# SpectacularAI/HybVIO

Measured on AMD Instinct MI355X. Metric: VIO frames/sec at 752x480 stereo, 200 KLT features; pyramid+KLT HBM GB/s, higher is better.
Workload: dtype u8/int16 pixels, int32/int64 sums, f32 solve (tracker); f64 (EKF); 1 GPU; C3: 752x480 stereo, 200 pts -- the whole frame chained on one stream per sequence: 2 pyramid builds, temporal LK from predicted positions, 2-point rotation RANSAC on its output, stereo LK, GFTT key points every 2nd frame (HIP tracker), then the HIP EKF from the device mean: 20 track visits (triangulation + prepareVisualUpdate + chi2 gate; track lengths 5 + Geometric(0.2) <= 21 stereo poses = 20 .~; sequences_per_gpu=4096, engines_per_gpu=4, parallelism=replicas x1 (no collective)

## Files before the change

hybvio_amd/csrc/rot_ransac.hip:

```cpp
#include "hv_camera.hpp"
#include "hv_internal.hpp"

#include <algorithm>
#include <cmath>

namespace hv {
namespace {

constexpr int RT_MANY = 256;
constexpr int RT_FEW = 1024;
constexpr int MAX_PTS = 1024;
constexpr int HYP = 100;
constexpr int RT_SPLIT_GROUPS = 25, RT_SPLIT = 256;
static_assert(HYP % RT_SPLIT_GROUPS == 0, "whole groups of hypotheses");
constexpr size_t SPLIT_REC_BYTES = sizeof(int) * (2 * HYP + 4) + sizeof(float) * 9 * HYP;

struct RansacArgs {
    int max_points;
    const int *n_points;
    const float *c1, *c2;
    const int *pairs;
    const uint32_t *draws;
    const uint8_t *lk_status;
    int lk_tracked;
    float threshold_pow2;
    int *status;
    float *R;
    int *summary;
    unsigned char *split;
    hv_camera_model cam1, cam2;
};

__device__ void cross3(const double *a, const double *b, double *c)
{
    c[0] = a[1] * b[2] - a[2] * b[1]; c[1] = a[2] * b[0] - a[0] * b[2]; c[2] = a[0] * b[1] - a[1] * b[0];
}

template <int P, int Q>
__device__ __forceinline__ void jacobi_step(double *A, double *V)
{
    const double apq = A[3 * P + Q];
    if (apq == 0.0) return;
    const double theta = (A[3 * Q + Q] - A[3 * P + P]) / (2.0 * apq);
    const double t = (theta >= 0.0 ? 1.0 : -1.0) / (fabs(theta) + sqrt(theta * theta + 1.0));
    const double c = 1.0 / sqrt(t * t + 1.0), s = t * c;
#pragma unroll
    for (int k = 0; k < 3; ++k) {
        const double akp = A[3 * k + P], akq = A[3 * k + Q];
        A[3 * k + P] = c * akp - s * akq; A[3 * k + Q] = s * akp + c * akq;
    }
#pragma unroll
    for (int k = 0; k < 3; ++k) {
        const double apk = A[3 * P + k], aqk = A[3 * Q + k];
        A[3 * P + k] = c * apk - s * aqk; A[3 * Q + k] = s * apk + c * aqk;
    }
#pragma unroll
    for (int k = 0; k < 3; ++k) {
        const double vkp = V[3 * k + P], vkq = V[3 * k + Q];
        V[3 * k + P] = c * vkp - s * vkq; V[3 * k + Q] = s * vkp + c * vkq;
    }
}

__device__ void kabsch_rotation(const float *Hf, float *Rf)
{
    double H[9], A[9], V[9] = {1, 0, 0, 0, 1, 0, 0, 0, 1};
#pragma unroll
    for (int k = 0; k < 9; ++k) H[k] = (double)Hf[k];
#pragma unroll
    for (int r = 0; r < 3; ++r)
#pragma unroll
        for (int c = 0; c < 3; ++c) A[3 * r + c] = H[r] * H[c] + H[3 + r] * H[3 + c] + H[6 + r] * H[6 + c];
    for (int sweep = 0; sweep < 8; ++sweep) { jacobi_step<0, 1>(A, V); jacobi_step<0, 2>(A, V); jacobi_step<1, 2>(A, V); }
    const double e0 = A[0], e1 = A[4], e2 = A[8];
    int i0 = 0;
    if (e1 > e0) i0 = 1;
    if (e2 > (i0 == 0 ? e0 : e1)) i0 = 2;
    auto eig = [&](int i) { return i == 0 ? e0 : i == 1 ? e1 : e2; };
    int i1 = i0 == 0 ? 1 : 0;
#pragma unroll
    for (int k = 0; k < 3; ++k) if (k != i0 && eig(k) > eig(i1)) i1 = k;
    auto col = [&](int i, int r) { return i == 0 ? V[3 * r] : i == 1 ? V[3 * r + 1] : V[3 * r + 2]; };
    const double v1[3] = {col(i0, 0), col(i0, 1), col(i0, 2)}, v2[3] = {col(i1, 0), col(i1, 1), col(i1, 2)};
    double v3[3], u1[3], u2[3], u3[3];
    const double l1 = eig(i0), l2 = eig(i1);
    const double s1 = sqrt(l1 > 0 ? l1 : 0.0), s2 = sqrt(l2 > 0 ? l2 : 0.0);
#pragma unroll
    for (int r = 0; r < 3; ++r) {
        u1[r] = H[3 * r] * v1[0] + H[3 * r + 1] * v1[1] + H[3 * r + 2] * v1[2];
        u2[r] = H[3 * r] * v2[0] + H[3 * r + 1] * v2[1] + H[3 * r + 2] * v2[2];
    }
    if (s1 > 0.0) {
#pragma unroll
        for (int r = 0; r < 3; ++r) u1[r] /= s1;
    } else { u1[0] = 1; u1[1] = 0; u1[2] = 0; }
    if (s2 > 1e-12 * s1 && s2 > 0.0) {
        const double d = u2[0] * u1[0] + u2[1] * u1[1] + u2[2] * u1[2];
#pragma unroll
        for (int r = 0; r < 3; ++r) u2[r] = u2[r] / s2 - (d / s2) * u1[r];
        const double nn = sqrt(u2[0] * u2[0] + u2[1] * u2[1] + u2[2] * u2[2]);
#pragma unroll
        for (int r = 0; r < 3; ++r) u2[r] /= nn;
    } else {
        int k0 = 0;
        if (fabs(u1[1]) < fabs(u1[0])) k0 = 1;
        if (fabs(u1[2]) < fabs(k0 == 0 ? u1[0] : u1[1])) k0 = 2;
        const double ax2[3] = {k0 == 0 ? 1.0 : 0.0, k0 == 1 ? 1.0 : 0.0, k0 == 2 ? 1.0 : 0.0};
        cross3(u1, ax2, u2);
        const double nn = sqrt(u2[0] * u2[0] + u2[1] * u2[1] + u2[2] * u2[2]);
#pragma unroll
        for (int r = 0; r < 3; ++r) u2[r] /= nn;
    }
    cross3(v1, v2, v3);
    cross3(u1, u2, u3);
#pragma unroll
    for (int r = 0; r < 3; ++r)
#pragma unroll
        for (int c = 0; c < 3; ++c) Rf[3 * r + c] = (float)(v1[r] * u1[c] + v2[r] * u2[c] + v3[r] * u3[c]);
}

__device__ bool inlier(const float *R, const float *p1, float c2x, float c2y, const hv_camera_model &cam2, double thr)
{
    float q[3];
#pragma unroll
    for (int r = 0; r < 3; ++r) {
        float s = 0.0f;
#pragma unroll
        for (int k = 0; k < 3; ++k) s = s + R[3 * r + k] * p1[k];
        q[r] = s;
    }
    const double ray[3] = {(double)q[0], (double)q[1], (double)q[2]};
    double pix[2];
    if (!ray_to_pixel(cam2, ray, pix)) return false;
    const float qx = (float)pix[0], qy = (float)pix[1];
    const double dx = (double)(c2x - qx), dy = (double)(c2y - qy);
    return dx * dx + dy * dy <= thr;
}

template <int RT, int NG = 1>
__global__ __launch_bounds__(RT) void rot_ransac_kernel(RansacArgs a)
{
    constexpr int HPG = HYP / NG;
    __shared__ float s_p1[MAX_PTS * 3], s_p2[MAX_PTS * 3], s_c2[MAX_PTS * 2];
    __shared__ float s_R[HYP * 9];
    __shared__ int s_count[HYP], s_valid[HYP];
    __shared__ unsigned char s_in[MAX_PTS];
    __shared__ float s_Rb[9];
    __shared__ int s_best[4];
    __shared__ unsigned short s_map[MAX_PTS];
    __shared__ int s_chunk[MAX_PTS / 64 + 1];
    const int set = NG > 1 ? blockIdx.y : blockIdx.x, tid = threadIdx.x;
    const int k_lo = NG > 1 ? (int)blockIdx.x * HPG : 0;
    const int n_all = min(max(a.n_points[set], 0), a.max_points);
    const float *c1 = a.c1 + (size_t)set * a.max_points * 2, *c2 = a.c2 + (size_t)set * a.max_points * 2;
    int *status = a.status + (size_t)set * a.max_points;
    int n = n_all;
    if (a.lk_status) {
        const uint8_t *ls = a.lk_status + (size_t)set * a.max_points;
        const int nchunk = (n_all + 63) / 64, wave = tid >> 6, lane = tid & 63;
        for (int ch = wave; ch < nchunk; ch += RT / 64) {
            const int i = ch * 64 + lane;
            const unsigned long long m = __ballot(i < n_all && ls[i] == a.lk_tracked);
            if (lane == 0) s_chunk[ch] = __popcll(m);
        }
        __syncthreads();
        if (tid == 0) {
            int acc = 0;
            for (int ch = 0; ch < nchunk; ++ch) { const int cnt = s_chunk[ch]; s_chunk[ch] = acc; acc += cnt; }
            s_chunk[nchunk] = acc;
        }
        __syncthreads();
        n = s_chunk[nchunk];
        for (int ch = wave; ch < nchunk; ch += RT / 64) {
            const int i = ch * 64 + lane;
            const bool on = i < n_all && ls[i] == a.lk_tracked;
            const unsigned long long m = __ballot(on);
            if (on) s_map[s_chunk[ch] + __popcll(m & ((1ull << lane) - 1ull))] = (unsigned short)i;
        }
    } else {
        for (int i = tid; i < n_all; i += RT) s_map[i] = (unsigned short)i;
    }
    __syncthreads();
    if (n < 2) {
        if (tid == 0 && k_lo == 0) { a.summary[2 * set] = 0; a.summary[2 * set + 1] = 0; }
        return;
    }
    const double thr = (double)a.threshold_pow2;
    for (int i = tid; i < n; i += RT) {
        const int src = s_map[i];
        double r[3];
        pixel_to_ray(a.cam1, (double)c1[2 * src], (double)c1[2 * src + 1], r);
        s_p1[3 * i] = (float)r[0]; s_p1[3 * i + 1] = (float)r[1]; s_p1[3 * i + 2] = (float)r[2];
        pixel_to_ray(a.cam2, (double)c2[2 * src], (double)c2[2 * src + 1], r);
        s_p2[3 * i] = (float)r[0]; s_p2[3 * i + 1] = (float)r[1]; s_p2[3 * i + 2] = (float)r[2];
        s_c2[2 * i] = c2[2 * src]; s_c2[2 * i + 1] = c2[2 * src + 1];
    }
    if (tid < HYP) s_count[tid] = 0;
    __syncthreads();
    if (tid < HPG) {
        const int hk = k_lo + tid;
        int i1, i2;
        if (a.draws) {
            i1 = (int)(a.draws[((size_t)set * HYP + hk) * 2] % (uint32_t)n);
            i2 = (int)(a.draws[((size_t)set * HYP + hk) * 2 + 1] % (uint32_t)n);
        } else {
            i1 = a.pairs[((size_t)set * HYP + hk) * 2]; i2 = a.pairs[((size_t)set * HYP + hk) * 2 + 1];
        }
        const int ok = i1 != i2 && (unsigned)i1 < (unsigned)n && (unsigned)i2 < (unsigned)n;
        s_valid[hk] = ok;
        if (ok) {
            float H[9] = {0, 0, 0, 0, 0, 0, 0, 0, 0}, R[9];
#pragma unroll
            for (int w = 0; w < 2; ++w) {
                const float *p = s_p1 + 3 * (w ? i2 : i1), *q = s_p2 + 3 * (w ? i2 : i1);
#pragma unroll
                for (int r = 0; r < 3; ++r)
#pragma unroll
                    for (int c = 0; c < 3; ++c) { const float prod = p[r] * q[c]; H[3 * r + c] = H[3 * r + c] + prod; }
            }
            kabsch_rotation(H, R);
#pragma unroll
            for (int k = 0; k < 9; ++k) s_R[9 * hk + k] = R[k];
        }
    }
    __syncthreads();
    for (int w = tid; w < n * HPG; w += RT) {
        const int kk = w / n, i = w - kk * n, k = k_lo + kk;
        if (s_valid[k] && inlier(s_R + 9 * k, s_p1 + 3 * i, s_c2[2 * i], s_c2[2 * i + 1], a.cam2, thr)) atomicAdd(&s_count[k], 1);
    }
    __syncthreads();
    if constexpr (NG > 1) {
        int *rec_i = reinterpret_cast<int *>(a.split + (size_t)set * SPLIT_REC_BYTES);
        float *rec_R = reinterpret_cast<float *>(rec_i + 2 * HYP + 4);
        if (tid < HPG) {
            rec_i[k_lo + tid] = s_count[k_lo + tid];
            rec_i[HYP + k_lo + tid] = s_valid[k_lo + tid];
        }
        for (int i = tid; i < 9 * HPG; i += RT) rec_R[9 * k_lo + i] = s_valid[k_lo + i / 9] ? s_R[9 * k_lo + i] : 0.0f;
        __threadfence();
        __syncthreads();
        if (tid == 0) s_best[3] = atomicAdd(&rec_i[2 * HYP], 1);
        __syncthreads();
        if (s_best[3] != NG - 1) return;
        __threadfence();
        if (tid < HYP) {
            s_count[tid] = __hip_atomic_load(&rec_i[tid], __ATOMIC_RELAXED, __HIP_MEMORY_SCOPE_AGENT);
            s_valid[tid] = __hip_atomic_load(&rec_i[HYP + tid], __ATOMIC_RELAXED, __HIP_MEMORY_SCOPE_AGENT);
        }
        for (int i = tid; i < 9 * HYP; i += RT) s_R[i] = __hip_atomic_load(&rec_R[i], __ATOMIC_RELAXED, __HIP_MEMORY_SCOPE_AGENT);
        if (tid == 0) rec_i[2 * HYP] = 0;
        __syncthreads();
    }
    if (tid == 0) {
        int best = 0, bk = -1, visited = HYP;
        for (int k = 0; k < HYP; ++k) {
            if (!s_valid[k]) continue;
            if (s_count[k] > best) { best = s_count[k]; bk = k; }
            if (s_count[k] == n) { visited = k + 1; break; }
        }
        s_best[0] = best; s_best[1] = bk; s_best[2] = visited;
        a.summary[2 * set] = best; a.summary[2 * set + 1] = visited;
        float R[9];
        if (bk >= 0) {
#pragma unroll
            for (int k = 0; k < 9; ++k) R[k] = s_R[9 * bk + k];
        } else {
            float H[9] = {0, 0, 0, 0, 0, 0, 0, 0, 0};
#pragma unroll
            for (int w = 0; w < 2; ++w)
#pragma unroll
                for (int r = 0; r < 3; ++r)
#pragma unroll
                    for (int c = 0; c < 3; ++c) { const float prod = s_p1[3 * w + r] * s_p2[3 * w + c]; H[3 * r + c] = H[3 * r + c] + prod; }
            kabsch_rotation(H, R);
        }
#pragma unroll
        for (int k = 0; k < 9; ++k) s_Rb[k] = R[k];
    }
    __syncthreads();
    for (int i = tid; i < n; i += RT) s_in[i] = inlier(s_Rb, s_p1 + 3 * i, s_c2[2 * i], s_c2[2 * i + 1], a.cam2, thr) ? 1 : 0;
    __syncthreads();
    if (tid < 64) {
        const int r = tid / 3, c = tid - 3 * r;
        float h = 0.0f;
        int cnt = 0;
        if (tid < 9)
            for (int i = 0; i < n; ++i)
                if (s_in[i]) { const float prod = s_p1[3 * i + r] * s_p2[3 * i + c]; h = h + prod; ++cnt; }
        float H[9];
#pragma unroll
        for (int k = 0; k < 9; ++k) H[k] = __shfl(h, k);
        if (tid == 0 && cnt >= 2) {
            float R[9];
            kabsch_rotation(H, R);
#pragma unroll
            for (int k = 0; k < 9; ++k) s_Rb[k] = R[k];
        }
    }
    __syncthreads();
    for (int i = tid; i < n; i += RT) status[s_map[i]] = inlier(s_Rb, s_p1 + 3 * i, s_c2[2 * i], s_c2[2 * i + 1], a.cam2, thr) ? 0 : 3;
    if (tid < 9) a.R[9 * (size_t)set + tid] = s_Rb[tid];
}

}
}

using hv::Ctx;

namespace hv {
int rot_ransac_alloc_split(Ctx *c)
{
    if (c->d_ransac_split) return HV_OK;
    const int sets = std::max(16, c->num_cus / RT_SPLIT_GROUPS);
    if (c->d_ransac_split.alloc(SPLIT_REC_BYTES * (size_t)sets)) return HV_ERR_NOMEM;
    HV_HIP(c, hipMemsetAsync(c->d_ransac_split, 0, SPLIT_REC_BYTES * (size_t)sets, c->stream));
    c->ransac_split_sets = sets;
    return HV_OK;
}
}

extern "C" {

int hv_camera_model_init(hv_camera_model *m)
{
    if (!m || (m->kind != 0 && m->kind != 1) || m->n_coeffs < 0 || m->n_coeffs > 4) return HV_ERR_INVALID;
    const double K[9] = {m->fx, 0, m->ppx, 0, m->fy, m->ppy, 0, 0, 1};
    {
        const double c00 = K[4] * K[8] - K[5] * K[7], c01 = K[5] * K[6] - K[3] * K[8], c02 = K[3] * K[7] - K[4] * K[6];
        const double det = K[0] * c00 + K[1] * c01 + K[2] * c02, id = 1.0 / det;
        double *o = m->kinv;
        o[0] = c00 * id; o[1] = (K[2] * K[7] - K[1] * K[8]) * id; o[2] = (K[1] * K[5] - K[2] * K[4]) * id;
        o[3] = c01 * id; o[4] = (K[0] * K[8] - K[2] * K[6]) * id; o[5] = (K[2] * K[3] - K[0] * K[5]) * id;
        o[6] = c02 * id; o[7] = (K[1] * K[6] - K[0] * K[7]) * id; o[8] = (K[0] * K[4] - K[1] * K[3]) * id;
    }
    m->n_table = 0; m->max_theta = m->max_r = 0;
    if (m->kind == 0) {
        m->distortion_enabled = !(m->n_coeffs == 0 || (m->n_coeffs == 1 && m->coeffs[0] == 0.)) ? 1 : 0;
        if (m->distortion_enabled && m->n_coeffs != 3) return HV_ERR_INVALID;
        if (m->rotation_enabled) {
            double d = 0;
            for (int i = 0; i < 9; ++i) { const double e = m->rotation[i] - (i % 4 == 0 ? 1.0 : 0.0); d += e * e; }
            m->rotation_enabled = std::sqrt(d) > 1e-8 ? 1 : 0;
        }
        return HV_OK;
    }
    m->rotation_enabled = 0;
    m->distortion_enabled = m->n_coeffs > 1 ? 1 : 0;
    if (m->distortion_enabled && m->n_coeffs != 4) return HV_ERR_INVALID;
    auto distort = [&](double theta, double *der) {
        if (!m->distortion_enabled) { if (der) *der = 1.0; return theta; }
        const double *k = m->coeffs, t = theta, t2 = t * t;
        if (der) *der = 1 + 3 * t2 * (k[0] + 5.0 / 3 * t2 * (k[1] + 7.0 / 5 * t2 * (k[2] + 9.0 / 7 * t2 * k[3])));
        return t * (1 + t2 * (k[0] + t2 * (k[1] + t2 * (k[2] + t2 * k[3]))));
    };
    m->max_theta = 0.5 * m->max_valid_fov_deg / 180.0 * M_PI;
    m->max_r = distort(m->max_theta, nullptr);
    if (m->distortion_enabled) {
        const double eps = 0.01 / ((m->fx + m->fy) * 0.5), step = m->max_r / 50.0;
        double theta = 0;
        for (int i = 0; i < 50; ++i) {
            const double r = (i + 0.5) * step;
            double th = theta, d, res = -1;
            for (int it = 0; it < 20; ++it) {
                const double dr = distort(th, &d) - r, dt = dr / d;
                th -= dt;
                if (std::fabs(dt) < eps) { res = th > 0.0 ? th : 0.0; break; }
            }
            if (res < 0) return HV_ERR_INVALID;
            m->table[m->n_table++] = res;
            theta = res + step;
        }
    }
    return HV_OK;
}

namespace hv { namespace {
int launch_rot_ransac(Ctx *c, int n_sets, RansacArgs &a)
{
    const int rt_forced = c->knob.rot_ransac_threads;
    const bool split = (rt_forced == RT_SPLIT_GROUPS || (rt_forced == 0 && n_sets * RT_SPLIT_GROUPS <= c->num_cus)) && n_sets <= c->ransac_split_sets;
    if (split) {
        a.split = c->d_ransac_split;
        hipLaunchKernelGGL((rot_ransac_kernel<RT_SPLIT, RT_SPLIT_GROUPS>), dim3(RT_SPLIT_GROUPS, (unsigned)n_sets), dim3(RT_SPLIT), 0, c->stream, a);
    } else if (rt_forced == RT_FEW || (rt_forced != RT_MANY && n_sets <= 64))
        hipLaunchKernelGGL((rot_ransac_kernel<RT_FEW>), dim3((unsigned)n_sets), dim3(RT_FEW), 0, c->stream, a);
    else
        hipLaunchKernelGGL((rot_ransac_kernel<RT_MANY>), dim3((unsigned)n_sets), dim3(RT_MANY), 0, c->stream, a);
    HV_HIP(c, hipGetLastError());
    return HV_OK;
}
} }

int hv_rot_ransac_batch_dev(hv_ctx *h, int n_sets, int max_points, const int *n_points_dev, const float *c1_dev, const float *c2_dev,
                            const hv_camera_model *cam1, const hv_camera_model *cam2, const int *pairs_dev, float threshold_pow2,
                            int *status_dev, float *R_dev, int *summary_dev)
{
    Ctx *c = hv::ctx_of(h);
    if (!c || n_sets < 0 || max_points < 2 || max_points > hv::MAX_PTS || !cam1 || !cam2) return HV_ERR_INVALID;
    if (n_sets > 0 && (!n_points_dev || !c1_dev || !c2_dev || !pairs_dev || !status_dev || !R_dev || !summary_dev)) return HV_ERR_INVALID;
    if (n_sets == 0) return HV_OK;
    hv::RansacArgs a{};
    a.max_points = max_points; a.n_points = n_points_dev; a.c1 = c1_dev; a.c2 = c2_dev; a.pairs = pairs_dev;
    a.threshold_pow2 = threshold_pow2; a.status = status_dev; a.R = R_dev; a.summary = summary_dev;
    a.cam1 = *cam1; a.cam2 = *cam2;
    hv::ScopedKernelTime tm(c, HV_K_ROT_RANSAC);
    return hv::launch_rot_ransac(c, n_sets, a);
}

int hv_rot_ransac_lk_batch_dev(hv_ctx *h, int n_sets, int max_points, const int *n_points_dev, const float *c1_dev, const float *c2_dev,
                               const uint8_t *lk_status_dev, int lk_tracked_value, const hv_camera_model *cam1,
                               const hv_camera_model *cam2, const uint32_t *draws_dev, float threshold_pow2, int *status_dev,
                               float *R_dev, int *summary_dev)
{
    Ctx *c = hv::ctx_of(h);
    if (!c || n_sets < 0 || max_points < 2 || max_points > hv::MAX_PTS || !cam1 || !cam2) return HV_ERR_INVALID;
    if (n_sets > 0 && (!n_points_dev || !c1_dev || !c2_dev || !lk_status_dev || !draws_dev || !status_dev || !R_dev || !summary_dev))
        return HV_ERR_INVALID;
    if (n_sets == 0) return HV_OK;
    hv::RansacArgs a{};
    a.max_points = max_points; a.n_points = n_points_dev; a.c1 = c1_dev; a.c2 = c2_dev; a.draws = draws_dev;
    a.lk_status = lk_status_dev; a.lk_tracked = lk_tracked_value;
    a.threshold_pow2 = threshold_pow2; a.status = status_dev; a.R = R_dev; a.summary = summary_dev;
    a.cam1 = *cam1; a.cam2 = *cam2;
    hv::ScopedKernelTime tm(c, HV_K_ROT_RANSAC);
    return hv::launch_rot_ransac(c, n_sets, a);
}

int hv_rot_ransac(hv_ctx *h, int n, const float *c1, const float *c2, const hv_camera_model *cam1, const hv_camera_model *cam2,
                  const int *pairs, float threshold_pow2, int *status, float *R, int *best_inlier_count, int *hypotheses_visited)
{
    Ctx *c = hv::ctx_of(h);
    if (!c || n < 2 || n > hv::MAX_PTS || !c1 || !c2 || !pairs || !status || !cam1 || !cam2) return HV_ERR_INVALID;
    hv::Stage s(c);
    const auto o_c1 = s.take<float>(2 * (size_t)n), o_c2 = s.take<float>(2 * (size_t)n), o_R = s.take<float>(9);
    const auto o_pairs = s.take<int>(2 * hv::HYP), o_n = s.take<int>(1), o_st = s.take<int>(n), o_sum = s.take<int>(2);
    int rc = s.reserve();
    if (rc != HV_OK) return rc;
    float *d_c1 = s.at(o_c1), *d_c2 = s.at(o_c2), *d_R = s.at(o_R);
    int *d_pairs = s.at(o_pairs), *d_n = s.at(o_n), *d_st = s.at(o_st), *d_sum = s.at(o_sum);
    HV_HIP(c, hipMemcpyAsync(d_c1, c1, sizeof(float) * 2 * n, hipMemcpyHostToDevice, c->stream));
    HV_HIP(c, hipMemcpyAsync(d_c2, c2, sizeof(float) * 2 * n, hipMemcpyHostToDevice, c->stream));
    HV_HIP(c, hipMemcpyAsync(d_pairs, pairs, sizeof(int) * 2 * hv::HYP, hipMemcpyHostToDevice, c->stream));
    HV_HIP(c, hipMemcpyAsync(d_n, &n, sizeof(int), hipMemcpyHostToDevice, c->stream));
    rc = hv_rot_ransac_batch_dev(h, 1, n, d_n, d_c1, d_c2, cam1, cam2, d_pairs, threshold_pow2, d_st, d_R, d_sum);
    if (rc != HV_OK) return rc;
    int summary[2] = {0, 0};
    HV_HIP(c, hipMemcpyAsync(status, d_st, sizeof(int) * n, hipMemcpyDeviceToHost, c->stream));
    if (R) HV_HIP(c, hipMemcpyAsync(R, d_R, sizeof(float) * 9, hipMemcpyDeviceToHost, c->stream));
    HV_HIP(c, hipMemcpyAsync(summary, d_sum, sizeof(summary), hipMemcpyDeviceToHost, c->stream));
    HV_HIP(c, hipStreamSynchronize(c->stream));
    if (best_inlier_count) *best_inlier_count = summary[0];
    if (hypotheses_visited) *hypotheses_visited = summary[1];
    return HV_OK;
}

}
```

Measured before the change: 155,300 frames/s.

## Add float fast-path inlier test, dynamic LDS sizing, and wave-level RANSAC reductions

Adds a float-only pinhole/polynomial projection test with a rigorous error bound that decides inlier/outlier directly and falls back to the double-precision path only for borderline cases. Shared memory for per-point arrays is now sized dynamically from max_points, which can raise occupancy for 200-point sets. Hypothesis counting uses wave ballots to aggregate atomics, best-hypothesis selection becomes a wave-wide max reduction, and the refit H accumulation iterates a compacted inlier list. The cost is more code complexity and reliance on the error bound being correct so results stay bit-identical to the double path.

```diff
diff --git a/hybvio_amd/csrc/rot_ransac.hip b/hybvio_amd/csrc/rot_ransac.hip
--- a/hybvio_amd/csrc/rot_ransac.hip
+++ b/hybvio_amd/csrc/rot_ransac.hip
@@ -136,17 +136,79 @@
     return dx * dx + dy * dy <= thr;
 }
 
+constexpr float FAST_ZMIN = 0x1p-10f, FAST_R2MAX = 2.0f, FAST_U = 0x1p-24f;
+
+struct FastCam {
+    float fx, fy, ppx, ppy, k0, k1, k2, e1x, e1y, e0x, e0y, thr;
+    bool on;
+};
+
+__device__ FastCam fast_cam(const hv_camera_model &c, float thr)
+{
+    FastCam f;
+    const bool d = c.distortion_enabled != 0;
+    f.fx = (float)c.fx; f.fy = (float)c.fy; f.ppx = (float)c.ppx; f.ppy = (float)c.ppy;
+    f.k0 = d ? (float)c.coeffs[0] : 0.0f; f.k1 = d ? (float)c.coeffs[1] : 0.0f; f.k2 = d ? (float)c.coeffs[2] : 0.0f;
+    const float tm = 1.0f + FAST_R2MAX * (fabsf(f.k0) + FAST_R2MAX * (fabsf(f.k1) + FAST_R2MAX * fabsf(f.k2)));
+    f.e1x = 128.0f * FAST_U * fabsf(f.fx) * tm; f.e1y = 128.0f * FAST_U * fabsf(f.fy) * tm;
+    f.e0x = 8.0f * FAST_U * fabsf(f.ppx) + 0x1p-100f; f.e0y = 8.0f * FAST_U * fabsf(f.ppy) + 0x1p-100f;
+    f.thr = thr;
+    f.on = c.kind == 0 && f.e1x + f.e1y + f.e0x + f.e0y < 1.0f;
+    return f;
+}
+
+__device__ __forceinline__ bool inlier_fast(const FastCam &f, const float *R, const float *p1, float c2x, float c2y, const hv_camera_model &cam2,
+                                            double thr)
+{
+    float q[3];
+#pragma unroll
+    for (int r = 0; r < 3; ++r) {
+        float s = 0.0f;
+#pragma unroll
+        for (int k = 0; k < 3; ++k) s = s + R[3 * r + k] * p1[k];
+        q[r] = s;
+    }
+    if (f.on) {
+        float r0 = q[0], r1 = q[1], z = q[2];
+        if (cam2.rotation_enabled) {
+            const double *Rc = cam2.rotation, a0 = (double)q[0], a1 = (double)q[1], a2 = (double)q[2];
+            r0 = (float)(Rc[0] * a0 + Rc[3] * a1 + Rc[6] * a2); r1 = (float)(Rc[1] * a0 + Rc[4] * a1 + Rc[7] * a2);
+            z = (float)(Rc[2] * a0 + Rc[5] * a1 + Rc[8] * a2);
+        }
+        if (z > FAST_ZMIN) {
+            const float iz = __builtin_amdgcn_rcpf(z), x = r0 * iz, y = r1 * iz, r2 = __builtin_fmaf(x, x, y * y);
+            if (r2 < FAST_R2MAX) {
+                const float th = __builtin_fmaf(r2, __builtin_fmaf(r2, __builtin_fmaf(r2, f.k2, f.k1), f.k0), 1.0f);
+                const float dx = c2x - __builtin_fmaf(f.fx, x * th, f.ppx), dy = c2y - __builtin_fmaf(f.fy, y * th, f.ppy);
+                const float D = __builtin_fmaf(dx, dx, dy * dy);
+                const float ex = __builtin_fmaf(f.e1x, fabsf(x), f.e0x), ey = __builtin_fmaf(f.e1y, fabsf(y), f.e0y);
+                const float B = __builtin_fmaf(2.0f * ex, fabsf(dx) + ex, __builtin_fmaf(2.0f * ey, fabsf(dy) + ey, 16.0f * FAST_U * D));
+                if (D + B < f.thr) return true;
+                if (D - B > f.thr) return false;
+            }
+        }
+    }
+    return inlier(R, p1, c2x, c2y, cam2, thr);
+}
+
+constexpr size_t RT_LDS_PER_POINT = 37;
+static_assert(RT_LDS_PER_POINT * MAX_PTS <= 48 * 1024, "the carve stays below the default dynamic-LDS limit");
+inline size_t rot_ransac_lds_bytes(int max_points) { return RT_LDS_PER_POINT * (size_t)((max_points + 3) & ~3); }
+
 template <int RT, int NG = 1>
 __global__ __launch_bounds__(RT) void rot_ransac_kernel(RansacArgs a)
 {
     constexpr int HPG = HYP / NG;
-    __shared__ float s_p1[MAX_PTS * 3], s_p2[MAX_PTS * 3], s_c2[MAX_PTS * 2];
+    extern __shared__ float s_dyn[];
+    const int P = (a.max_points + 3) & ~3;
+    float *const s_p1 = s_dyn, *const s_p2 = s_p1 + 3 * P, *const s_c2 = s_p2 + 3 * P;
+    unsigned short *const s_map = reinterpret_cast<unsigned short *>(s_c2 + 2 * P);
+    unsigned short *const s_list = s_map + P;
+    unsigned char *const s_in = reinterpret_cast<unsigned char *>(s_list + P);
     __shared__ float s_R[HYP * 9];
     __shared__ int s_count[HYP], s_valid[HYP];
-    __shared__ unsigned char s_in[MAX_PTS];
     __shared__ float s_Rb[9];
     __shared__ int s_best[4];
-    __shared__ unsigned short s_map[MAX_PTS];
     __shared__ int s_chunk[MAX_PTS / 64 + 1];
     const int set = NG > 1 ? blockIdx.y : blockIdx.x, tid = threadIdx.x;
     const int k_lo = NG > 1 ? (int)blockIdx.x * HPG : 0;
@@ -185,6 +247,10 @@
         return;
     }
     const double thr = (double)a.threshold_pow2;
+    const FastCam fc = fast_cam(a.cam2, a.threshold_pow2);
+    auto test = [&](const float *R, int i) {
+        return inlier_fast(fc, R, s_p1 + 3 * i, s_c2[2 * i], s_c2[2 * i + 1], a.cam2, thr);
+    };
     for (int i = tid; i < n; i += RT) {
         const int src = s_map[i];
         double r[3];
@@ -223,9 +289,22 @@
         }
     }
     __syncthreads();
-    for (int w = tid; w < n * HPG; w += RT) {
-        const int kk = w / n, i = w - kk * n, k = k_lo + kk;
-        if (s_valid[k] && inlier(s_R + 9 * k, s_p1 + 3 * i, s_c2[2 * i], s_c2[2 * i + 1], a.cam2, thr)) atomicAdd(&s_count[k], 1);
+    {
+        const int total = n * HPG, dq = RT / n, dr = RT - dq * n, lane = tid & 63;
+        int kk = tid / n, i = tid - kk * n;
+        for (int base = 0; base < total; base += RT) {
+            const int k = k_lo + kk;
+            const bool hit = base + tid < total && s_valid[k] && test(s_R + 9 * k, i);
+            unsigned long long pending = __ballot(hit);
+            while (pending) {
+                const int leader = __ffsll(pending) - 1, kl = __shfl(k, leader);
+                const unsigned long long m = __ballot(hit && k == kl);
+                if (lane == leader) atomicAdd(&s_count[kl], __popcll(m));
+                pending &= ~m;
+            }
+            kk += dq; i += dr;
+            if (i >= n) { i -= n; ++kk; }
+        }
     }
     __syncthreads();
     if constexpr (NG > 1) {
@@ -250,21 +329,23 @@
         if (tid == 0) rec_i[2 * HYP] = 0;
         __syncthreads();
     }
-    if (tid == 0) {
-        int best = 0, bk = -1, visited = HYP;
-        for (int k = 0; k < HYP; ++k) {
-            if (!s_valid[k]) continue;
-            if (s_count[k] > best) { best = s_count[k]; bk = k; }
-            if (s_count[k] == n) { visited = k + 1; break; }
-        }
-        s_best[0] = best; s_best[1] = bk; s_best[2] = visited;
-        a.summary[2 * set] = best; a.summary[2 * set + 1] = visited;
-        float R[9];
+    static_assert(HYP > 64 && HYP <= 128, "two hypotheses per lane");
+    if (tid < 64) {
+        const int ka = tid, kb = tid + 64;
+        const int ca = s_valid[ka] ? s_count[ka] : -1, cb = kb < HYP && s_valid[kb] ? s_count[kb] : -1;
+        const unsigned long long fa = __ballot(ca == n), fb = __ballot(cb == n);
+        const int first = fa ? __ffsll(fa) - 1 : fb ? 64 + __ffsll(fb) - 1 : HYP;
+        int key = 0;
+        if (ca > 0 && ka <= first) key = (ca << 7) | (127 - ka);
+        if (cb > 0 && kb <= first) key = max(key, (cb << 7) | (127 - kb));
+#pragma unroll
+        for (int d = 32; d; d >>= 1) key = max(key, __shfl_xor(key, d));
+        const int best = key >> 7, bk = key ? 127 - (key & 127) : -1;
+        if (tid == 0) { a.summary[2 * set] = best; a.summary[2 * set + 1] = first < HYP ? first + 1 : HYP; }
         if (bk >= 0) {
-#pragma unroll
-            for (int k = 0; k < 9; ++k) R[k] = s_R[9 * bk + k];
-        } else {
-            float H[9] = {0, 0, 0, 0, 0, 0, 0, 0, 0};
+            if (tid < 9) s_Rb[tid] = s_R[9 * bk + tid];
+        } else if (tid == 0) {
+            float H[9] = {0, 0, 0, 0, 0, 0, 0, 0, 0}, R[9];
 #pragma unroll
             for (int w = 0; w < 2; ++w)
 #pragma unroll
@@ -272,20 +353,40 @@
 #pragma unroll
                     for (int c = 0; c < 3; ++c) { const float prod = s_p1[3 * w + r] * s_p2[3 * w + c]; H[3 * r + c] = H[3 * r + c] + prod; }
             kabsch_rotation(H, R);
-        }
-#pragma unroll
-        for (int k = 0; k < 9; ++k) s_Rb[k] = R[k];
-    }
-    __syncthreads();
-    for (int i = tid; i < n; i += RT) s_in[i] = inlier(s_Rb, s_p1 + 3 * i, s_c2[2 * i], s_c2[2 * i + 1], a.cam2, thr) ? 1 : 0;
+#pragma unroll
+            for (int k = 0; k < 9; ++k) s_Rb[k] = R[k];
+        }
+    }
+    __syncthreads();
+    for (int i = tid; i < n; i += RT) s_in[i] = test(s_Rb, i) ? 1 : 0;
     __syncthreads();
     if (tid < 64) {
-        const int r = tid / 3, c = tid - 3 * r;
+        int cnt = 0;
+        for (int b = 0; b < n; b += 64) {
+            const int i = b + tid;
+            const bool on = i < n && s_in[i];
+            const unsigned long long m = __ballot(on);
+            if (on) s_list[cnt + __popcll(m & ((1ull << tid) - 1ull))] = (unsigned short)i;
+            cnt += __popcll(m);
+        }
+        if (tid == 0) s_best[0] = cnt;
+    }
+    __syncthreads();
+    if (tid < 64) {
+        const int cnt = s_best[0], r = tid / 3, c = tid - 3 * r;
         float h = 0.0f;
-        int cnt = 0;
-        if (tid < 9)
-            for (int i = 0; i < n; ++i)
-                if (s_in[i]) { const float prod = s_p1[3 * i + r] * s_p2[3 * i + c]; h = h + prod; ++cnt; }
+        if (tid < 9) {
+            const float *pr = s_p1 + r, *qc = s_p2 + c;
+            int j = 0;
+            for (; j + 8 <= cnt; j += 8) {
+                float prod[8];
+#pragma unroll
+                for (int u = 0; u < 8; ++u) { const int i = s_list[j + u]; prod[u] = pr[3 * i] * qc[3 * i]; }
+#pragma unroll
+                for (int u = 0; u < 8; ++u) h = h + prod[u];
+            }
+            for (; j < cnt; ++j) { const int i = s_list[j]; const float prod = pr[3 * i] * qc[3 * i]; h = h + prod; }
+        }
         float H[9];
 #pragma unroll
         for (int k = 0; k < 9; ++k) H[k] = __shfl(h, k);
@@ -297,7 +398,7 @@
         }
     }
     __syncthreads();
-    for (int i = tid; i < n; i += RT) status[s_map[i]] = inlier(s_Rb, s_p1 + 3 * i, s_c2[2 * i], s_c2[2 * i + 1], a.cam2, thr) ? 0 : 3;
+    for (int i = tid; i < n; i += RT) status[s_map[i]] = test(s_Rb, i) ? 0 : 3;
     if (tid < 9) a.R[9 * (size_t)set + tid] = s_Rb[tid];
 }
 
@@ -378,13 +479,14 @@
 {
     const int rt_forced = c->knob.rot_ransac_threads;
     const bool split = (rt_forced == RT_SPLIT_GROUPS || (rt_forced == 0 && n_sets * RT_SPLIT_GROUPS <= c->num_cus)) && n_sets <= c->ransac_split_sets;
+    const size_t lds = rot_ransac_lds_bytes(a.max_points);
     if (split) {
         a.split = c->d_ransac_split;
-        hipLaunchKernelGGL((rot_ransac_kernel<RT_SPLIT, RT_SPLIT_GROUPS>), dim3(RT_SPLIT_GROUPS, (unsigned)n_sets), dim3(RT_SPLIT), 0, c->stream, a);
+        hipLaunchKernelGGL((rot_ransac_kernel<RT_SPLIT, RT_SPLIT_GROUPS>), dim3(RT_SPLIT_GROUPS, (unsigned)n_sets), dim3(RT_SPLIT), lds, c->stream, a);
     } else if (rt_forced == RT_FEW || (rt_forced != RT_MANY && n_sets <= 64))
-        hipLaunchKernelGGL((rot_ransac_kernel<RT_FEW>), dim3((unsigned)n_sets), dim3(RT_FEW), 0, c->stream, a);
+        hipLaunchKernelGGL((rot_ransac_kernel<RT_FEW>), dim3((unsigned)n_sets), dim3(RT_FEW), lds, c->stream, a);
     else
-        hipLaunchKernelGGL((rot_ransac_kernel<RT_MANY>), dim3((unsigned)n_sets), dim3(RT_MANY), 0, c->stream, a);
+        hipLaunchKernelGGL((rot_ransac_kernel<RT_MANY>), dim3((unsigned)n_sets), dim3(RT_MANY), lds, c->stream, a);
     HV_HIP(c, hipGetLastError());
     return HV_OK;
 }
```

Result: no change. 156,100 frames/s, median of 4 (+0.6%).
